# nep-pack/NonlinearEigenproblems.jl

Measured on AMD Instinct MI355X. Metric: eigenpairs/sec (gun SPMF iar m=100) + compute_Mlincomb GB/s, higher is better.
Workload: dtype f64 (complex128)

## Files before the change

include/nepmi355.h:

```cpp
#ifndef NEPMI355_H
#define NEPMI355_H

#include <stddef.h>
#include <stdint.h>

#ifdef __cplusplus
extern "C" {
#endif

typedef struct { double re, im; } nep_cdouble;
typedef struct nep_spmf nep_spmf;
typedef struct nep_lu nep_lu;
typedef struct nep_comm nep_comm;
typedef void* nep_stream;

#define NEP_OK 0
#define NEP_ERR_HIP -1
#define NEP_ERR_ARG -2
#define NEP_ERR_SINGULAR -3
#define NEP_ERR_BREAKDOWN -4
#define NEP_ERR_UNSUPPORTED -5
#define NEP_ERR_RETRY -6
#define NEP_ERR_NOCONV -7

// ... 261 lines not shown
    double tol;
    double neigs;
    nep_cdouble sigma, gamma;
} nep_iar_opts;
typedef struct nep_iar_result {
    int32_t k;
    int32_t nconv;
    int32_t nret;
    int32_t refine_plan;
    int32_t refine_hint_off;
    int32_t retry_reason;
} nep_iar_result;
typedef int32_t (*nep_fv_eval)(void* ctx, int32_t nlam, const nep_cdouble* lam, nep_cdouble* F);
int32_t nep_refine_review(int32_t umfpack_refinements, int32_t plan, int32_t final_recorded, const double* w4, int32_t hint_in,
                          int32_t out[4]);
int32_t nep_iar_run(nep_spmf* spmf, nep_lu* lu, int64_t n, const nep_iar_opts* opts, const nep_cdouble* h_v0,
                    const nep_cdouble* h_Ctab, int32_t mt, const double* h_cabs, const nep_cdouble* h_cf, const double* h_fro,
                    nep_fv_eval fv, void* ctx, nep_cdouble* h_lam, nep_cdouble* dQ, nep_cdouble* h_Q, double* h_err,
                    nep_cdouble* dV_basis, nep_iar_result* res, nep_stream stream);

int32_t nep_comm_unique_id(void* h_out128);
int32_t nep_comm_create(int32_t rank, int32_t world, const void* h_unique_id128, nep_comm** out);
int32_t nep_comm_destroy(nep_comm* c);
int32_t nep_comm_info(const nep_comm* c, int32_t out[2]);
int32_t nep_allgather_sum(nep_comm* c, const nep_cdouble* d_partial, int64_t len, nep_cdouble* d_total, nep_stream stream);
int32_t nep_sum_ranks(const nep_cdouble* d_parts, int64_t len, int32_t world, nep_cdouble* d_total, nep_stream stream);

#ifdef __cplusplus
}
#endif
// ... 2 lines not shown
```

nonlineareigenproblems.jl_amd/_lib.py:

```python
import ctypes as C
import os

import numpy as np
import torch

from ._env import env_flag

_HERE = os.path.dirname(os.path.abspath(__file__))
LIB_PATH = os.path.join(_HERE, "libnepmi355.so")


class NepError(RuntimeError):
    def __init__(self, status, msg):
        super().__init__("libnepmi355 status %d: %s" % (status, msg))
        self.status = status


NEP_OK, NEP_ERR_HIP, NEP_ERR_ARG, NEP_ERR_SINGULAR, NEP_ERR_BREAKDOWN, NEP_ERR_UNSUPPORTED = 0, -1, -2, -3, -4, -5
NEP_ERR_RETRY, NEP_ERR_NOCONV = -6, -7


def _load():
    from . import build
    if build.needs_build():
# ... 124 lines not shown
    "nep_lu_refac_destroy": [c_vp],
    "nep_lu_refac_info": [c_vp, c_vp],
    "nep_lu_refac_wide_info": [c_vp, c_vp],
    "nep_lu_refac_hash": [c_vp, c_vp],
    "nep_lu_factor_dev": [c_vp, c_vp, c_i32, C.c_double, c_vp, c_vp, c_vp, c_vp],
    "nep_lu_refac_analyze": [c_i64, c_vp, c_vp, c_vp, c_vp, c_vp, c_vp, c_vp, c_vp, c_vp],
    "nep_lu_factor_dev_batch": [c_vp, c_i32, c_vp, c_i32, C.c_double, c_vp, c_vp, c_vp, c_vp],
    "nep_lu_factor_dev_batch_terms": [c_vp, c_i32, c_vp, c_i32, c_vp, c_i32, C.c_double, c_vp, c_vp, c_vp],
    "nep_iar_step": [c_vp, c_i32, c_i32, c_vp],
    "nep_iar_steps": [c_vp, c_i32, c_i32, c_i32, c_vp],
    "nep_iar_wait": [c_vp, c_i32],
    "nep_iar_stream_wait": [c_vp, c_i32, c_vp],
    "nep_devprim_exclusive_sum": [c_vp, c_vp, c_i64, c_vp],
    "nep_devprim_sort_pairs": [c_vp, c_vp, c_i64, c_i32, c_vp],
    "nep_refine_review": [c_i32, c_i32, c_i32, c_vp, c_i32, c_vp],
    "nep_iar_run": [c_vp, c_vp, c_i64, c_vp, c_vp, c_vp, c_i32, c_vp, c_vp, c_vp, c_vp, c_vp, c_vp, c_vp, c_vp, c_vp, c_vp, c_vp, c_vp],
    "nep_hess_eig_worksize": [c_i32, P(c_i64)],
    "nep_hess_eigvals_dev": [c_i32, c_vp, c_i64, c_vp, c_vp, c_vp, c_vp],
    "nep_hess_eigvecs_dev": [c_i32, c_vp, c_vp, c_i64, c_vp, c_vp, c_vp],
    "nep_hess_eigvals_batch_dev": [c_i32, c_i32, c_i32, c_vp, c_i64, c_vp, c_i64, c_vp, c_i64, c_vp, c_i64, c_vp],
    "nep_hess_eigvecs_batch_dev": [c_i32, c_i32, c_i32, c_vp, c_i64, c_vp, c_i64, c_i64, c_vp, c_i64, c_vp, c_i64, c_vp],
    "nep_comm_unique_id": [c_vp],
    "nep_comm_create": [c_i32, c_i32, c_vp, P(c_vp)],
    "nep_comm_destroy": [c_vp],
    "nep_comm_info": [c_vp, P(c_i32)],
    "nep_allgather_sum": [c_vp, c_vp, c_i64, c_vp, c_vp],
    "nep_sum_ranks": [c_vp, c_i64, c_i32, c_vp, c_vp],
    "nep_iar_shift_scale": [c_i64, c_i32, c_vp, c_vp, c_vp],
    "nep_rk_bw": [c_i64, c_i32, c_vp, c_vp, c_vp, c_vp],
    "nep_discretize_polygon": [c_i32, c_vp, c_i32, c_vp],
# ... 64 lines not shown
```

nonlineareigenproblems.jl_amd/csrc/driver.hip:

```cpp
#include "common.h"
#include <vector>
#include <stdlib.h>
#include <time.h>

struct nep_iar {
    nep_spmf* spmf; nep_lu* lu;
    int64_t n, ldv; int32_t m, mt;
    cplx* dV; const cplx* dCtab; int64_t ldc; const int64_t* d_active;
    cplx* dz; cplx* dW;
    std::vector<double> cabs; std::vector<nep_cdouble> cf;
    cplx* dH; nep_cdouble* hH;
    double* d_cabs; cplx* d_ccf;
    cplx* hH_dev;
    int32_t method;
    std::vector<hipEvent_t> ev;
    hipEvent_t e_upload = nullptr; bool upload_waited = false;
    hipStream_t last = nullptr;
    bool no_events = false;
    std::vector<hipGraphExec_t> graphs;
    cplx* dWT = nullptr; int32_t wt_for = 0;
};

extern "C" {

int32_t nep_iar_create(nep_spmf* spmf, nep_lu* lu, int64_t n, int32_t m, nep_cdouble* dV, int64_t ldv,
                       const nep_cdouble* dCtab, int64_t ldc, const int64_t* d_active, nep_cdouble* dwork3n,
                       const double* h_cabs, const nep_cdouble* h_cf, int32_t mt, nep_cdouble* dH, nep_cdouble* h_pinnedH,
                       int32_t orth_method, nep_iar** out) {
    ARGCHK(out != nullptr);
    *out = nullptr;
// ... 95 lines not shown
        if (rc) return rc;
    }
    cplx* mirror = s->hH_dev ? s->hH_dev + (int64_t)(k - 1) * (s->m + 4) : nullptr;
    if (s->dWT && k < s->m) {
        rc = nep_orth_dev_iar_next((const nep_cdouble*)s->dV, s->ldv, n, k, s->d_active, (nep_cdouble*)vv, (nep_cdouble*)hrow, s->method,
                                   (nep_cdouble*)mirror, k + 4, (const nep_cdouble*)s->dCtab, s->ldc, s->mt,
                                   (nep_cdouble*)s->dWT, (nep_cdouble*)(vv + s->ldv + n), stream);
        if (!rc) s->wt_for = k + 1;
    } else
        rc = nep_orth_dev_mirror((const nep_cdouble*)s->dV, s->ldv, n * (int64_t)(k + 1), k, s->d_active, (nep_cdouble*)vv,
                                 (nep_cdouble*)hrow, s->method, (nep_cdouble*)mirror, k + 4, stream);
    if (rc) return rc;
    if (!mirror)
        HIPCHK(hipMemcpyAsync(s->hH + (int64_t)(k - 1) * (s->m + 4), hrow, (size_t)(k + 4) * sizeof(cplx), hipMemcpyDeviceToHost, st));
    if (s->no_events) return NEP_OK;
    if (!s->ev[k]) HIPCHK(hipEventCreateWithFlags(&s->ev[k], hipEventDisableTiming | hipEventBlockingSync));
    HIPCHK(hipEventRecord(s->ev[k], st));
    return NEP_OK;
}

int32_t nep_iar_steps(nep_iar* s, int32_t k0, int32_t count, int32_t refine_steps, nep_stream stream) {
    ARGCHK(s && count >= 1);
    for (int32_t k = k0; k < k0 + count; ++k) {
        int rc = nep_iar_step(s, k, refine_steps, stream);
        if (rc) return rc;
    }
    return NEP_OK;
}

int32_t nep_iar_steps_graph(nep_iar* s, int32_t k0, int32_t count, int32_t refine_steps, nep_stream stream, int32_t* captured) {
    ARGCHK(s && count >= 1);
    if (captured) *captured = 0;
// ... 8 lines not shown
        hipGraph_t g = nullptr;
        hipError_t e = hipStreamEndCapture(st, &g);
        hipGraphExec_t ge = nullptr;
        if (!rc && e == hipSuccess && g && hipGraphInstantiate(&ge, g, nullptr, nullptr, 0) == hipSuccess && ge) {
            if (hipGraphLaunch(ge, st) == hipSuccess) { s->graphs.push_back(ge); ok = true; }
            else (void)hipGraphExecDestroy(ge);
        }
        if (g) (void)hipGraphDestroy(g);
        if (!ok) (void)hipGetLastError();
    } else (void)hipGetLastError();
    if (!ok) {
        s->wt_for = wt_for0; s->upload_waited = waited0; s->last = last0;
        return nep_iar_steps(s, k0, count, refine_steps, stream);
    }
    for (int32_t k = k0; k < k0 + count; ++k) {
        if (!s->ev[k]) HIPCHK(hipEventCreateWithFlags(&s->ev[k], hipEventDisableTiming | hipEventBlockingSync));
        HIPCHK(hipEventRecord(s->ev[k], st));
    }
    if (captured) *captured = 1;
    return NEP_OK;
}

int32_t nep_iar_wait(nep_iar* s, int32_t k) {
    ARGCHK(s && k >= 1 && k <= s->m && s->ev[k]);
    for (;;) {
        const hipError_t e = hipEventQuery(s->ev[k]);
        if (e == hipSuccess) return NEP_OK;
        if (e != hipErrorNotReady) HIPCHK(e);
        struct timespec ts = {0, 20000};
        nanosleep(&ts, nullptr);
// ... 11 lines not shown
```

nonlineareigenproblems.jl_amd/csrc/iar_run.hip:

```cpp
#include "common.h"
#include <algorithm>
#include <deque>
#include <map>
#include <mutex>
#include <vector>
#include <math.h>
#include <time.h>

extern "C" {
int32_t nep_iar_create(nep_spmf* spmf, nep_lu* lu, int64_t n, int32_t m, nep_cdouble* dV, int64_t ldv, const nep_cdouble* dCtab,
                       int64_t ldc, const int64_t* d_active, nep_cdouble* dwork3n, const double* h_cabs, const nep_cdouble* h_cf,
                       int32_t mt, nep_cdouble* dH, nep_cdouble* h_pinnedH, int32_t orth_method, nep_iar** out);
int32_t nep_iar_steps_graph(nep_iar* s, int32_t k0, int32_t count, int32_t refine_steps, nep_stream stream, int32_t* captured);
}

namespace {

constexpr double EPS = 2.220446049250313e-16;

__global__ void k_iar_active(int64_t* act, int64_t n, int m1) {
    const int j = blockIdx.x * blockDim.x + threadIdx.x;
    if (j < m1) act[j] = (int64_t)(j + 1) * n;
}
__global__ void k_iar_start(cplx* __restrict__ V, const cplx* __restrict__ v, double inv, int64_t n) {
    const int64_t i = (int64_t)blockIdx.x * blockDim.x + threadIdx.x;
    if (i < n) V[i] = cmake(v[i].x * inv, v[i].y * inv);
}

// ... 40 lines not shown
    RunStreams& r = g_rs[dev];
    if (!r.check || !r.eig || r.probed_for != main || (r.shared && r.retries < 3)) {
        if (r.shared) ++r.retries;
        r.shared = false;
        int rc = pick_stream(r.check, {main}, &r.check, &r.shared); if (rc) return rc;
        rc = pick_stream(r.eig, {main, r.check}, &r.eig, &r.shared); if (rc) return rc;
        r.probed_for = main;
    }
    *out = r;
    return NEP_OK;
}

struct Arena {
    int dev = -1; int64_t n = 0; int32_t m = 0, mt = 0;
    cplx* Hdev = nullptr; cplx* wdev = nullptr; cplx* Ctab = nullptr; cplx* work3n = nullptr; int64_t* active = nullptr;
    cplx* v0 = nullptr; double* d_norms = nullptr; void* eigwork = nullptr; int64_t wsz = 0; int bmax = 0;
    cplx* Hpin = nullptr; cplx* wpin = nullptr; double* npin = nullptr; cplx* stage = nullptr;
    void release() {
        for (void* p : {(void*)Hdev, (void*)wdev, (void*)Ctab, (void*)work3n, (void*)active, (void*)v0, (void*)d_norms, eigwork})
            if (p) nep_pool_free(p);
        for (void* p : {(void*)Hpin, (void*)wpin, (void*)npin, (void*)stage}) if (p) (void)hipHostFree(p);
        *this = Arena();
    }
};
std::mutex g_arena_mu;
std::vector<Arena> g_arenas;

int arena_acquire(int64_t n, int32_t m, int32_t mt, int bmax, Arena* out) {
    int dev = 0; HIPCHK(hipGetDevice(&dev));
    {
        std::lock_guard<std::mutex> lk(g_arena_mu);
        for (size_t i = 0; i < g_arenas.size(); ++i)
            if (g_arenas[i].dev == dev && g_arenas[i].n == n && g_arenas[i].m == m && g_arenas[i].mt == mt && g_arenas[i].bmax == bmax) {
                *out = g_arenas[i]; g_arenas.erase(g_arenas.begin() + i); return NEP_OK;
            }
    }
    Arena a; a.dev = dev; a.n = n; a.m = m; a.mt = mt; a.bmax = bmax;
    int64_t wsz = 0; int rc = nep_hess_eig_worksize(m, &wsz); if (rc) return rc;
    a.wsz = (wsz + 15) / 16 * 16;
    void* p = nullptr;
#define AL(dst, type, bytes) do { rc = nep_pool_alloc(&p, (size_t)(bytes)); if (rc) { a.release(); return rc; } dst = (type)p; } while (0)
    AL(a.Hdev, cplx*, (size_t)m * (m + 4) * 16);
    AL(a.wdev, cplx*, (size_t)m * (m + 2) * 16);
    AL(a.Ctab, cplx*, (size_t)m * mt * 16);
    AL(a.work3n, cplx*, (size_t)3 * n * 16);
    AL(a.active, int64_t*, (size_t)(m + 1) * 8);
    AL(a.v0, cplx*, (size_t)n * 16);
    AL(a.d_norms, double*, (size_t)m * 2 * m * 8);
    AL(a.eigwork, void*, (size_t)bmax * a.wsz);
#undef AL
    const size_t stage_bytes = std::max<size_t>((size_t)n * 16, (size_t)m * mt * 16);
    if (hipHostMalloc((void**)&a.Hpin, (size_t)m * (m + 4) * 16, hipHostMallocMapped) != hipSuccess ||
        hipHostMalloc((void**)&a.wpin, (size_t)m * (m + 2) * 16, hipHostMallocMapped) != hipSuccess ||
        hipHostMalloc((void**)&a.npin, (size_t)m * 2 * m * 8, hipHostMallocDefault) != hipSuccess ||
        hipHostMalloc((void**)&a.stage, stage_bytes, hipHostMallocDefault) != hipSuccess) {
        (void)hipGetLastError(); a.release();
        nep_set_error("nep_iar_run: pinned host allocation failed");
        return NEP_ERR_HIP;
    }
    *out = a;
    return NEP_OK;
}
void arena_return(Arena& a) {
    std::lock_guard<std::mutex> lk(g_arena_mu);
// ... 29 lines not shown
            const double om = w[step];
            if (om <= 2.0 * EPS) { ret = step; break; }
            if (om > 0.5 * w_prev) { ret = om > w_prev ? step - 1 : step; break; }
            if (step == umf) { ret = step; break; }
            w_prev = om;
        }
        if (ret < 0) ret = plan;
        last_omega = w[plan];
        recorded = std::max(ret, 1);
        const bool ok = isfinite(w[plan]) && (ret == plan || w[plan] <= std::max(4.0 * EPS, w[ret]));
        if (ok) { if (!hint_off) hint = recorded; } else { hint = -1; hint_off = true; }
        return ok;
    }
};

struct Batch { std::vector<int> kcs; cplx* Zb = nullptr; int kmax = 0; hipEvent_t evW = nullptr, evZ = nullptr; };
struct Check { int kc = 0; std::vector<double> lam; cplx* QT = nullptr; std::vector<double> F; hipEvent_t ev = nullptr; cplx* Zb_owner = nullptr; };

inline cplx hc(const nep_cdouble& z) { cplx r; r.x = z.re; r.y = z.im; return r; }
inline bool ev_done(hipEvent_t e) {
    if (hipEventQuery(e) == hipSuccess) return true;
    (void)hipGetLastError();
    return false;
}

struct Run {
    nep_spmf* spmf; nep_lu* lu; int64_t n; nep_iar_opts o; nep_fv_eval fv; void* ctx; const double* h_fro;
    hipStream_t st; RunStreams rs; Arena a; bool have_arena = false;
    int32_t m, mt; int64_t ldv;
    cplx* V = nullptr; bool own_V = true; nep_iar* step = nullptr;
    Refine ref;
    std::vector<char> filled; std::vector<int> plans;
    std::vector<hipEvent_t> ev_pool;
    std::vector<double> s_lam; std::vector<int> s_idx; cplx* s_QT = nullptr; int s_kq = 0; int conv = 0; int k_checked = 0;
    std::vector<double> s_err;
    double* h_err = nullptr;
    int retry = 0;

    hipEvent_t event() {
        if (!ev_pool.empty()) { hipEvent_t e = ev_pool.back(); ev_pool.pop_back(); return e; }
        hipEvent_t e = nullptr;
        if (hipEventCreateWithFlags(&e, hipEventDisableTiming) != hipSuccess) { (void)hipGetLastError(); return nullptr; }
        return e;
    }
    void done(hipEvent_t e) { if (e) ev_pool.push_back(e); }

    int fail_kind = 0, fail_at = 0;
    int fill_H(int kk) {
        for (int j = 1; j <= kk; ++j) {
            if (filled[j]) continue;
            if (fail_at == j && (fail_kind == 1 || fail_kind == 2)) {
                retry = fail_kind; nep_set_error("nep_iar_run: injected miss of kind %d at step %d", fail_kind, j); return NEP_ERR_RETRY;
// ... 5 lines not shown
            if (ref.umf > 0) {
                const int plan = plans[j];
                const bool final_rec = !((plan & 0x100) && (j % 8) != 0);
                if (!ref.review((const double*)(row + j + 2), plan & 0xff, final_rec)) {
                    retry = 1; nep_set_error("nep_iar_run: the refinement record of step %d asks for more sweeps than were taken", j);
                    return NEP_ERR_RETRY;
                }
            }
            filled[j] = 1;
        }
        return NEP_OK;
    }
    ~Run() {
        if (step) (void)nep_iar_destroy(step);
        if (V && own_V) nep_pool_free_on(V, st, true);
        if (s_QT) nep_pool_free_on(s_QT, rs.check, true);
        for (hipEvent_t e : ev_pool) (void)hipEventDestroy(e);
        if (have_arena) arena_return(a);
    }
};

}

extern "C" {

int32_t nep_refine_review(int32_t umfpack_refinements, int32_t plan, int32_t final_recorded, const double* w4, int32_t hint_in,
                          int32_t out[4]) {
    ARGCHK(w4 && out && plan >= 0 && plan <= 3 && umfpack_refinements >= 0);
    Refine r; r.umf = umfpack_refinements; r.hint = hint_in;
    const bool ok = r.review(w4, plan, final_recorded != 0);
    out[0] = ok ? 1 : 0; out[1] = r.recorded; out[2] = r.hint; out[3] = r.hint_off ? 1 : 0;
    return NEP_OK;
}

int32_t nep_iar_run(nep_spmf* spmf, nep_lu* lu, int64_t n, const nep_iar_opts* opts, const nep_cdouble* h_v0,
                    const nep_cdouble* h_Ctab, int32_t mt, const double* h_cabs, const nep_cdouble* h_cf, const double* h_fro,
                    nep_fv_eval fv, void* ctx, nep_cdouble* h_lam, nep_cdouble* dQ, nep_cdouble* h_Q, double* h_err,
                    nep_cdouble* dV_basis, nep_iar_result* res, nep_stream stream) {
    ARGCHK(spmf && lu && opts && h_v0 && h_Ctab && fv && h_lam && res);
    ARGCHK(n > 0 && mt >= 1 && opts->maxit >= 1 && opts->check_error_every >= 1);
    ARGCHK(opts->orth_method == 0 || opts->orth_method == 1);
    ARGCHK(opts->errmeasure == 0 || (opts->errmeasure == 1 && h_fro));
    ARGCHK(opts->umfpack_refinements <= 0 || (h_cabs && h_cf));
    memset(res, 0, sizeof(*res));
    res->refine_plan = -1;
    struct timespec t_e_; clock_gettime(CLOCK_MONOTONIC, &t_e_);
    const double t_entry = t_e_.tv_sec * 1e3 + t_e_.tv_nsec * 1e-6;
    const int32_t m = opts->maxit;
    if (m > 128) { nep_set_error("nep_iar_run: maxit = %d exceeds the device eigen-decomposition's limit 128", m); return NEP_ERR_UNSUPPORTED; }
    const int BMAX = std::max(1, nep_env_int("NEP_IAR_EIG_BATCH", 16));
    const int LASTB = std::max(1, nep_env_int("NEP_IAR_EIG_LAST", 8));
    const double T100 = nep_env_double("NEP_IAR_EIG_MS100", 3.3);
    const double TSTEP = 0.35;
    const int cee = opts->check_error_every;
    const double neigs = opts->neigs;
    const bool unthrottled = isinf(neigs) && neigs > 0;

    Run R; R.spmf = spmf; R.lu = lu; R.n = n; R.o = *opts; R.fv = fv; R.ctx = ctx; R.h_fro = h_fro; R.st = as_stream(stream);
    R.m = m; R.mt = mt; R.ldv = n * (int64_t)(m + 1); R.h_err = h_err;
    int rc = run_streams(R.st, &R.rs); if (rc) return rc;
    rc = arena_acquire(n, m, mt, BMAX, &R.a); if (rc) return rc;
    R.have_arena = true;
    Arena& a = R.a;
    hipStream_t st = R.st, cst = R.rs.check, est = R.rs.eig;
    R.ref.umf = opts->umfpack_refinements > 0 ? opts->umfpack_refinements : 0;
    R.ref.hint = (opts->refine_hint >= 0 && nep_env_int("NEP_REFINE_HINT", 1) != 0) ? opts->refine_hint : -1;
    R.filled.assign(m + 1, 0); R.plans.assign(m + 1, 0);
    if (const char* fa = getenv("NEP_IAR_RUN_FAIL_AT")) { if (sscanf(fa, "%d:%d", &R.fail_kind, &R.fail_at) != 2) R.fail_kind = R.fail_at = 0; }
    if (h_err) for (int64_t i = 0; i < (int64_t)m * m; ++i) h_err[i] = NAN;

    if (dV_basis) { R.V = (cplx*)dV_basis; R.own_V = false; }
    else {
        void* p = nullptr;
        rc = nep_pool_alloc(&p, (size_t)(m + 1) * R.ldv * 16); if (rc) return rc;
        R.V = (cplx*)p;
    }
// ... 12 lines not shown
    HIPCHK(hipMemsetAsync(a.Hdev, 0, (size_t)m * (m + 4) * 16, st));
    LAUNCHCHK();
    memset(a.Hpin, 0, (size_t)m * (m + 4) * 16);
    memset(a.wpin, 0, (size_t)m * (m + 2) * 16);
    {
        static thread_local PinnedRing ring;
        rc = ring.upload(a.Ctab, h_Ctab, (size_t)m * mt * 16, st); if (rc) return rc;
    }
    rc = nep_iar_create(spmf, lu, n, m, (nep_cdouble*)R.V, R.ldv, (const nep_cdouble*)a.Ctab, m, a.active, (nep_cdouble*)a.work3n,
                        R.ref.umf > 0 ? h_cabs : nullptr, R.ref.umf > 0 ? h_cf : nullptr, mt, (nep_cdouble*)a.Hdev,
                        (nep_cdouble*)a.Hpin, opts->orth_method, &R.step);
    if (rc) return rc;

    std::vector<char> plan_end(m + 2, 0);
    if (unthrottled) {
        std::vector<int> allk;
        for (int kk = 1; kk <= m; ++kk) if (kk % cee == 0 || kk == m) allk.push_back(kk);
        int e_ = (int)allk.size(); int size = std::min(LASTB, e_);
        while (e_ > 0) {
            plan_end[allk[e_ - 1]] = 1; e_ -= size;
            if (e_ > 0) {
                const double q = allk[e_ - 1] / 100.0;
                size = (int)std::min<double>(std::min(BMAX, e_), std::max(1.0, ceil(2.0 * T100 * q * q / (TSTEP * cee))));
            }
        }
    }
    const bool trace = getenv("NEP_IAR_RUN_TRACE") != nullptr;
    auto now = []() { struct timespec t; clock_gettime(CLOCK_MONOTONIC, &t); return t.tv_sec * 1e3 + t.tv_nsec * 1e-6; };
    double t_fv = 0;
    std::deque<int> pendA; std::deque<Batch> stA; std::deque<Check> stC;
    int slots = unthrottled ? m + 1 : std::max(BMAX, 4);
    const int CHUNK = unthrottled ? 8 : 4;
    const int P = std::min(256, std::max(1, 3072 / mt));
    int k = 1; bool done = false; int status = NEP_OK;
    const bool use_graph = nep_env_flag("NEP_IAR_GRAPH");
    int n_graph = 0;
    auto finished = [&]() { return R.conv >= neigs; };

    auto batch_ready = [&]() -> int {
        if (pendA.empty()) return 0;
        int cnt = 1;
        while (cnt < (int)pendA.size() && cnt < BMAX && pendA[cnt] - pendA[cnt - 1] == pendA[1] - pendA[0] && !(unthrottled && plan_end[pendA[cnt - 1]])) ++cnt;
        if (!unthrottled || plan_end[pendA[cnt - 1]] || cnt >= BMAX || done) return cnt;
        return 0;
    };
    auto launch_batch = [&](int count) -> int {
        Batch b;
        for (int i = 0; i < count; ++i) { b.kcs.push_back(pendA.front()); pendA.pop_front(); }
        const int k0 = b.kcs[0], nb = count; b.kmax = b.kcs.back();
        const int kstep = nb > 1 ? b.kcs[1] - k0 : 0;
        int r = nep_iar_stream_wait(R.step, b.kmax, (nep_stream)est); if (r) return r;
        cplx* wrow = a.wdev + (int64_t)(k0 - 1) * (m + 2);
        cplx* mrow = a.wpin + (int64_t)(k0 - 1) * (m + 2);
        r = nep_hess_eigvals_batch_dev(nb, k0, kstep, (const nep_cdouble*)a.Hdev, m + 4, (nep_cdouble*)wrow, (int64_t)kstep * (m + 2),
                                       a.eigwork, a.wsz, (nep_cdouble*)mrow, (int64_t)kstep * (m + 2), (nep_stream)est);
        if (r) return r;
        b.evW = R.event(); if (!b.evW) return NEP_ERR_HIP;
        HIPCHK(hipEventRecord(b.evW, est));
        void* pz = nullptr;
        r = nep_pool_alloc(&pz, (size_t)nb * b.kmax * b.kmax * 16); if (r) return r;
        b.Zb = (cplx*)pz;
        r = nep_hess_eigvecs_batch_dev(nb, k0, kstep, (nep_cdouble*)wrow, (int64_t)kstep * (m + 2), (nep_cdouble*)b.Zb, b.kmax,
                                       (int64_t)b.kmax * b.kmax, a.eigwork, a.wsz, (nep_cdouble*)mrow, (int64_t)kstep * (m + 2), (nep_stream)est);
        if (r) { nep_pool_free_on(b.Zb, est, true); return r; }
        b.evZ = R.event(); if (!b.evZ) return NEP_ERR_HIP;
        HIPCHK(hipEventRecord(b.evZ, est));
        stA.push_back(b);
        return NEP_OK;
    };
    auto launch_check = [&](const Batch& b, int bi, bool first_of_batch) -> int {
        const int kc = b.kcs[bi];
        int r = R.fill_H(kc); if (r) return r;
        const cplx* w = a.wpin + (int64_t)(kc - 1) * (m + 2);
        if (w[kc].x != 0.0 || (R.fail_kind == 3 && R.fail_at == kc)) { R.retry = 3; nep_set_error("nep_iar_run: the QR iteration of step %d gave up", kc); return NEP_ERR_RETRY; }
        Check c; c.kc = kc; c.lam.resize(2 * (size_t)kc); c.F.resize(2 * (size_t)mt * kc);
        const double sr = R.o.sigma.re, si = R.o.sigma.im, gr = R.o.gamma.re, gi = R.o.gamma.im;
        for (int s = 0; s < kc; ++s) {
            const double dr = w[s].x, di = w[s].y, den = dr * dr + di * di;
            c.lam[2 * s] = sr + (gr * dr + gi * di) / den;
            c.lam[2 * s + 1] = si + (gi * dr - gr * di) / den;
        }
        const double tf0 = trace ? now() : 0.0;
        const int32_t frc = R.fv(R.ctx, kc, (const nep_cdouble*)c.lam.data(), (nep_cdouble*)c.F.data());
        if (trace) t_fv += now() - tf0;
        if (frc != 0) {
            nep_set_error("nep_iar_run: the f_t(lambda) callback failed in step %d", kc); return NEP_ERR_ARG;
        }
        if (first_of_batch) HIPCHK(hipStreamWaitEvent(cst, b.evZ, 0));
        void* pq = nullptr;
        r = nep_pool_alloc(&pq, (size_t)n * kc * 16); if (r) return r;
        c.QT = (cplx*)pq;
        r = nep_gemm_ts_dev((const nep_cdouble*)R.V, R.ldv, n, kc, (const nep_cdouble*)(b.Zb + (int64_t)bi * b.kmax * b.kmax), b.kmax, 0, kc,
                            (nep_cdouble*)c.QT, kc, 1, (nep_stream)cst);
        double* d_out = a.d_norms + (int64_t)(kc - 1) * 2 * m;
        if (!r) r = nep_resid_batch_dev(spmf, kc, (const nep_cdouble*)c.F.data(), (const nep_cdouble*)c.QT, kc, d_out, (nep_stream)cst);
        if (r) { nep_pool_free_on(c.QT, cst, true); return r; }
        HIPCHK(hipMemcpyAsync(a.npin + (int64_t)(kc - 1) * 2 * m, d_out, (size_t)2 * kc * 8, hipMemcpyDeviceToHost, cst));
        c.ev = R.event(); if (!c.ev) return NEP_ERR_HIP;
        HIPCHK(hipEventRecord(c.ev, cst));
        if (bi == (int)b.kcs.size() - 1) c.Zb_owner = b.Zb;
        stC.push_back(std::move(c));
        return NEP_OK;
    };
    auto consume = [&](Check& c) -> int {
        const int kc = c.kc;
        const cplx* w = a.wpin + (int64_t)(kc - 1) * (m + 2);
        if (w[kc + 1].x != 0.0) { R.retry = 3; nep_set_error("nep_iar_run: an inverse iteration of step %d did not grow", kc); return NEP_ERR_RETRY; }
        const double* sq = a.npin + (int64_t)(kc - 1) * 2 * m;
        std::vector<double> e(kc);
        for (int j0 = 0; j0 < kc; j0 += P) {
            const int kk = std::min(P, kc - j0);
            for (int j = 0; j < kk; ++j) {
                const double rn = sqrt(sq[2 * j0 + j]), qn = sqrt(sq[2 * j0 + kk + j]);
                double den = qn;
                if (R.o.errmeasure == 1) {
// ... 11 lines not shown
        std::stable_sort(idx.begin(), idx.end(), [&](int x, int y) {
            const double ex = isnan(e[x]) ? INFINITY : e[x], ey = isnan(e[y]) ? INFINITY : e[y];
            return ex < ey;
        });
        R.s_err.assign(kc, 0.0);
        for (int s = 0; s < kc; ++s) R.s_err[s] = e[idx[s]];
        if (R.h_err) for (int s = 0; s < kc; ++s) R.h_err[(int64_t)s * m + (kc - 1)] = R.s_err[s];
        int nret = kc;
        if (kc == m || conv >= neigs) nret = (int)std::min<double>(kc, neigs);
        R.s_lam.resize(2 * (size_t)nret); R.s_idx.assign(idx.begin(), idx.begin() + nret);
        for (int s = 0; s < nret; ++s) {
            const int src = (kc == m || conv >= neigs) ? idx[s] : s;
            R.s_lam[2 * s] = c.lam[2 * src]; R.s_lam[2 * s + 1] = c.lam[2 * src + 1];
        }
        if (!(kc == m || conv >= neigs)) for (int s = 0; s < nret; ++s) R.s_idx[s] = idx[s];
        if (R.s_QT) nep_pool_free_on(R.s_QT, cst, true);
        R.s_QT = c.QT; c.QT = nullptr; R.s_kq = kc;
        R.conv = conv; R.k_checked = kc;
        R.done(c.ev); c.ev = nullptr;
        return NEP_OK;
    };
    auto drop_check = [&](Check& c) {
        if (c.QT) nep_pool_free_on(c.QT, cst, true);
        if (c.Zb_owner) nep_pool_free_on(c.Zb_owner, cst, true);
        R.done(c.ev);
    };
    auto drop_batch = [&](Batch& b) {
        if (b.Zb) nep_pool_free_on(b.Zb, est, true);
        R.done(b.evW); R.done(b.evZ);
    };

    hipEvent_t te0 = nullptr, te1 = nullptr; bool te1_rec = false;
    if (trace) { (void)hipEventCreate(&te0); (void)hipEventCreate(&te1); (void)hipEventRecord(te0, st); }
    const double t_loop = now();
    double tt_steps = 0, tt_A = 0, tt_B = 0, tt_C = 0, tt_sleep = 0, t_enq_done = 0; double tq = 0;
    while (status == NEP_OK) {
        bool progressed = false;
        tq = now();
        if (!done) {
            if (k <= m && !finished()) {
                int nb = 0;
                while (nb < CHUNK && k + nb <= m) {
                    const bool due = ((k + nb) % cee == 0) || (k + nb == m);
// ... 5 lines not shown
                    if (plan > 0 && R.ref.settled()) plan |= 0x100;
                    if (use_graph && k > 1) { int32_t cap = 0; status = nep_iar_steps_graph(R.step, k, nb, plan, stream, &cap); n_graph += cap; }
                    else status = nep_iar_steps(R.step, k, nb, plan, stream);
                    if (status) break;
                    for (int kk = k; kk < k + nb; ++kk) {
                        R.plans[kk] = plan;
                        if (kk % cee == 0 || kk == m) pendA.push_back(kk);
                    }
                    k += nb; progressed = true;
                }
            } else done = true;
            if (k > m) { if (!done && trace) { t_enq_done = now() - t_loop; if (te1 && !te1_rec) { (void)hipEventRecord(te1, st); te1_rec = true; } } done = true; }
        }
        if (trace) { const double t = now(); tt_steps += t - tq; tq = t; }
        while (!finished()) {
            const int cnt = batch_ready();
            if (!cnt) break;
            status = launch_batch(cnt); progressed = true;
            if (status) break;
        }
        if (status) break;
        if (trace) { const double t = now(); tt_A += t - tq; tq = t; }
        while (!stA.empty() && !finished() && ev_done(stA.front().evW)) {
            progressed = true;
            Batch b = stA.front(); stA.pop_front();
            for (int bi = 0; bi < (int)b.kcs.size() && status == NEP_OK; ++bi) {
                status = launch_check(b, bi, bi == 0);
                if (status == NEP_OK) ++slots;
            }
            if (status) { drop_batch(b); break; }
            R.done(b.evW); R.done(b.evZ);
        }
        if (status) break;
        if (trace) { const double t = now(); tt_B += t - tq; tq = t; }
        while (!stC.empty() && !finished() && ev_done(stC.front().ev)) {
            progressed = true;
            Check c = std::move(stC.front()); stC.pop_front();
            status = consume(c);
            if (c.Zb_owner) nep_pool_free_on(c.Zb_owner, cst, true);
            c.Zb_owner = nullptr;
            if (status) { drop_check(c); break; }
        }
        if (status) break;
        if (finished()) {
            done = true; pendA.clear();
            while (!stA.empty()) { drop_batch(stA.front()); stA.pop_front(); }
            while (!stC.empty()) { drop_check(stC.front()); stC.pop_front(); }
        }
        if (trace) { const double t = now(); tt_C += t - tq; tq = t; }
        if (done && pendA.empty() && stA.empty() && stC.empty()) break;
        if (!progressed) { struct timespec ts = {0, 20000}; nanosleep(&ts, nullptr); if (trace) { const double t = now(); tt_sleep += t - tq; tq = t; } }
    }
    if (trace)
        fprintf(stderr, "nep_iar_run trace (ms): set-up %.2f | loop %.2f: steps %.2f (all enqueued at %.2f) A %.2f B %.2f (callback %.2f) C %.2f sleep %.2f\n",
// ... 15 lines not shown
    res->refine_plan = R.ref.hint_off ? -1 : (R.ref.recorded >= 0 ? R.ref.recorded : R.ref.hint);
    res->refine_hint_off = R.ref.hint_off ? 1 : 0;
    if (status || !unthrottled) (void)hipStreamSynchronize(st);
    if (status) return status;

    int nret = (int)(R.s_lam.size() / 2);
    const bool noconv = (R.conv < neigs) && !unthrottled;
    if (!noconv) nret = std::min(nret, R.conv);
    res->k = R.k_checked > 0 ? R.k_checked : k - 1;
    res->nconv = R.conv; res->nret = nret;
    for (int s = 0; s < nret; ++s) { h_lam[s].re = R.s_lam[2 * s]; h_lam[s].im = R.s_lam[2 * s + 1]; }
    if (nret > 0 && (dQ || h_Q) && R.s_QT) {
        cplx* dst = (cplx*)dQ; void* tmp = nullptr;
        if (!dst) { rc = nep_pool_alloc(&tmp, (size_t)n * nret * 16); if (rc) return rc; dst = (cplx*)tmp; }
        std::vector<int32_t> cols(R.s_idx.begin(), R.s_idx.begin() + nret);
        rc = nep_rowmajor_to_colmajor(n, R.s_kq, (const nep_cdouble*)R.s_QT, R.s_kq, cols.data(), nret, (nep_cdouble*)dst, n, (nep_stream)cst);
        if (!rc && h_Q) {
            if (hipMemcpyAsync(h_Q, dst, (size_t)n * nret * 16, hipMemcpyDeviceToHost, cst) != hipSuccess) rc = NEP_ERR_HIP;
        }
        if (hipStreamSynchronize(cst) != hipSuccess && !rc) rc = NEP_ERR_HIP;
        if (tmp) nep_pool_free(tmp);
        if (rc) { if (rc == NEP_ERR_HIP) nep_set_error("nep_iar_run: returning the eigenvector block failed"); return rc; }
    }
    if (noconv) { nep_set_error("Number of iterations exceeded. maxit=%d.", m); return NEP_ERR_NOCONV; }
    return NEP_OK;
}

}
```

nonlineareigenproblems.jl_amd/csrc/util.hip:

```cpp
#include "common.h"
#include <vector>
#include <algorithm>
#include <math.h>
#include <time.h>

static thread_local char g_err[1024] = "";

void nep_set_error(const char* fmt, ...) {
    va_list ap;
    va_start(ap, fmt);
    vsnprintf(g_err, sizeof(g_err), fmt, ap);
    va_end(ap);
}

int NepScratch::ensure(size_t bytes) {
    if (bytes <= cap) return NEP_OK;
    if (dptr) { (void)hipDeviceSynchronize(); nep_pool_free(dptr); dptr = nullptr; cap = 0; }
    size_t want = std::max<size_t>(2 * bytes, (size_t)4 << 20);
    int rc = nep_pool_alloc(&dptr, want);
    if (rc) return rc;
    cap = want;
    return NEP_OK;
}
void NepScratch::release() {
// ... 97 lines not shown
        *p = busy_p;
        return NEP_OK;
    }
    {
        std::vector<PoolBlock> to_free;
        {
            std::lock_guard<std::mutex> lk(g_pool_mu);
            for (auto& kv : g_pool_free) to_free.push_back(kv.second);
            g_pool_free.clear(); g_pool_cached = 0;
        }
        pool_drop(to_free);
    }
    HIPCHK(hipMalloc(p, want));
    std::lock_guard<std::mutex> lk(g_pool_mu);
    g_pool_live[*p] = want;
    return NEP_OK;
}

void nep_pool_free(void* p) {
    if (!p) return;
    std::vector<PoolBlock> to_free;
    {
        std::lock_guard<std::mutex> lk(g_pool_mu);
        pool_put(p, nullptr, to_free);
    }
    pool_drop(to_free);
}

void nep_pool_free_on(void* p, hipStream_t st, bool in_flight) {
    if (!p) return;
// ... 643 lines not shown
```

Before: 1404.

## Run IAR eigen-check batches on alternating stream lanes with sparse step events

Eigenvalue/eigenvector batches and their residual checks now alternate between two stream lanes (eig and check), with the final step on the main stream. Each lane has its own eigen workspace slot, and event chaining orders the checks. Step events are recorded only at batch-end steps, and the batch plan splits off the last check. The aim is to let consecutive Hessenberg eig batches and residual checks overlap and to cut per-step event overhead. The cost is a larger workspace, more complex stream ordering, and a risk of ordering bugs.

```diff
diff --git a/include/nepmi355.h b/include/nepmi355.h
--- a/include/nepmi355.h
+++ b/include/nepmi355.h
@@ -299,6 +299,7 @@
 typedef int32_t (*nep_fv_eval)(void* ctx, int32_t nlam, const nep_cdouble* lam, nep_cdouble* F);
 int32_t nep_refine_review(int32_t umfpack_refinements, int32_t plan, int32_t final_recorded, const double* w4, int32_t hint_in,
                           int32_t out[4]);
+int32_t nep_iar_batch_plan(int32_t m, int32_t check_error_every, int32_t bmax, int32_t lastb, double ms100, char* out_end_flags);
 int32_t nep_iar_run(nep_spmf* spmf, nep_lu* lu, int64_t n, const nep_iar_opts* opts, const nep_cdouble* h_v0,
                     const nep_cdouble* h_Ctab, int32_t mt, const double* h_cabs, const nep_cdouble* h_cf, const double* h_fro,
                     nep_fv_eval fv, void* ctx, nep_cdouble* h_lam, nep_cdouble* dQ, nep_cdouble* h_Q, double* h_err,
diff --git a/nonlineareigenproblems.jl_amd/_lib.py b/nonlineareigenproblems.jl_amd/_lib.py
--- a/nonlineareigenproblems.jl_amd/_lib.py
+++ b/nonlineareigenproblems.jl_amd/_lib.py
@@ -162,6 +162,7 @@
     "nep_devprim_exclusive_sum": [c_vp, c_vp, c_i64, c_vp],
     "nep_devprim_sort_pairs": [c_vp, c_vp, c_i64, c_i32, c_vp],
     "nep_refine_review": [c_i32, c_i32, c_i32, c_vp, c_i32, c_vp],
+    "nep_iar_batch_plan": [c_i32, c_i32, c_i32, c_i32, C.c_double, c_vp],
     "nep_iar_run": [c_vp, c_vp, c_i64, c_vp, c_vp, c_vp, c_i32, c_vp, c_vp, c_vp, c_vp, c_vp, c_vp, c_vp, c_vp, c_vp, c_vp, c_vp, c_vp],
     "nep_hess_eig_worksize": [c_i32, P(c_i64)],
     "nep_hess_eigvals_dev": [c_i32, c_vp, c_i64, c_vp, c_vp, c_vp, c_vp],
diff --git a/nonlineareigenproblems.jl_amd/csrc/driver.hip b/nonlineareigenproblems.jl_amd/csrc/driver.hip
--- a/nonlineareigenproblems.jl_amd/csrc/driver.hip
+++ b/nonlineareigenproblems.jl_amd/csrc/driver.hip
@@ -14,6 +14,7 @@
     cplx* hH_dev;
     int32_t method;
     std::vector<hipEvent_t> ev;
+    std::vector<char> ev_wanted;
     hipEvent_t e_upload = nullptr; bool upload_waited = false;
     hipStream_t last = nullptr;
     bool no_events = false;
@@ -139,8 +140,15 @@
     if (!mirror)
         HIPCHK(hipMemcpyAsync(s->hH + (int64_t)(k - 1) * (s->m + 4), hrow, (size_t)(k + 4) * sizeof(cplx), hipMemcpyDeviceToHost, st));
     if (s->no_events) return NEP_OK;
+    if (!s->ev_wanted.empty() && !s->ev_wanted[k]) return NEP_OK;
     if (!s->ev[k]) HIPCHK(hipEventCreateWithFlags(&s->ev[k], hipEventDisableTiming | hipEventBlockingSync));
     HIPCHK(hipEventRecord(s->ev[k], st));
+    return NEP_OK;
+}
+
+int32_t nep_iar_event_steps(nep_iar* s, const char* wanted) {
+    ARGCHK(s);
+    if (wanted) s->ev_wanted.assign(wanted, wanted + s->m + 1); else s->ev_wanted.clear();
     return NEP_OK;
 }
 
@@ -179,6 +187,7 @@
         return nep_iar_steps(s, k0, count, refine_steps, stream);
     }
     for (int32_t k = k0; k < k0 + count; ++k) {
+        if (!s->ev_wanted.empty() && !s->ev_wanted[k]) continue;
         if (!s->ev[k]) HIPCHK(hipEventCreateWithFlags(&s->ev[k], hipEventDisableTiming | hipEventBlockingSync));
         HIPCHK(hipEventRecord(s->ev[k], st));
     }
diff --git a/nonlineareigenproblems.jl_amd/csrc/iar_run.hip b/nonlineareigenproblems.jl_amd/csrc/iar_run.hip
--- a/nonlineareigenproblems.jl_amd/csrc/iar_run.hip
+++ b/nonlineareigenproblems.jl_amd/csrc/iar_run.hip
@@ -12,6 +12,7 @@
                        int64_t ldc, const int64_t* d_active, nep_cdouble* dwork3n, const double* h_cabs, const nep_cdouble* h_cf,
                        int32_t mt, nep_cdouble* dH, nep_cdouble* h_pinnedH, int32_t orth_method, nep_iar** out);
 int32_t nep_iar_steps_graph(nep_iar* s, int32_t k0, int32_t count, int32_t refine_steps, nep_stream stream, int32_t* captured);
+int32_t nep_iar_event_steps(nep_iar* s, const char* wanted);
 }
 
 namespace {
@@ -82,7 +83,7 @@
 struct Arena {
     int dev = -1; int64_t n = 0; int32_t m = 0, mt = 0;
     cplx* Hdev = nullptr; cplx* wdev = nullptr; cplx* Ctab = nullptr; cplx* work3n = nullptr; int64_t* active = nullptr;
-    cplx* v0 = nullptr; double* d_norms = nullptr; void* eigwork = nullptr; int64_t wsz = 0; int bmax = 0;
+    cplx* v0 = nullptr; double* d_norms = nullptr; void* eigwork = nullptr; int64_t wsz = 0; int bmax = 0; int nslots = 0;
     cplx* Hpin = nullptr; cplx* wpin = nullptr; double* npin = nullptr; cplx* stage = nullptr;
     void release() {
         for (void* p : {(void*)Hdev, (void*)wdev, (void*)Ctab, (void*)work3n, (void*)active, (void*)v0, (void*)d_norms, eigwork})
@@ -94,16 +95,16 @@
 std::mutex g_arena_mu;
 std::vector<Arena> g_arenas;
 
-int arena_acquire(int64_t n, int32_t m, int32_t mt, int bmax, Arena* out) {
+int arena_acquire(int64_t n, int32_t m, int32_t mt, int bmax, int nslots, Arena* out) {
     int dev = 0; HIPCHK(hipGetDevice(&dev));
     {
         std::lock_guard<std::mutex> lk(g_arena_mu);
         for (size_t i = 0; i < g_arenas.size(); ++i)
-            if (g_arenas[i].dev == dev && g_arenas[i].n == n && g_arenas[i].m == m && g_arenas[i].mt == mt && g_arenas[i].bmax == bmax) {
+            if (g_arenas[i].dev == dev && g_arenas[i].n == n && g_arenas[i].m == m && g_arenas[i].mt == mt && g_arenas[i].bmax == bmax && g_arenas[i].nslots == nslots) {
                 *out = g_arenas[i]; g_arenas.erase(g_arenas.begin() + i); return NEP_OK;
             }
     }
-    Arena a; a.dev = dev; a.n = n; a.m = m; a.mt = mt; a.bmax = bmax;
+    Arena a; a.dev = dev; a.n = n; a.m = m; a.mt = mt; a.bmax = bmax; a.nslots = nslots;
     int64_t wsz = 0; int rc = nep_hess_eig_worksize(m, &wsz); if (rc) return rc;
     a.wsz = (wsz + 15) / 16 * 16;
     void* p = nullptr;
@@ -115,7 +116,7 @@
     AL(a.active, int64_t*, (size_t)(m + 1) * 8);
     AL(a.v0, cplx*, (size_t)n * 16);
     AL(a.d_norms, double*, (size_t)m * 2 * m * 8);
-    AL(a.eigwork, void*, (size_t)bmax * a.wsz);
+    AL(a.eigwork, void*, (size_t)nslots * a.wsz);
 #undef AL
     const size_t stage_bytes = std::max<size_t>((size_t)n * 16, (size_t)m * mt * 16);
     if (hipHostMalloc((void**)&a.Hpin, (size_t)m * (m + 4) * 16, hipHostMallocMapped) != hipSuccess ||
@@ -175,8 +176,28 @@
     }
 };
 
-struct Batch { std::vector<int> kcs; cplx* Zb = nullptr; int kmax = 0; hipEvent_t evW = nullptr, evZ = nullptr; };
-struct Check { int kc = 0; std::vector<double> lam; cplx* QT = nullptr; std::vector<double> F; hipEvent_t ev = nullptr; cplx* Zb_owner = nullptr; };
+struct Batch { std::vector<int> kcs; cplx* Zb = nullptr; int kmax = 0; hipEvent_t evW = nullptr, evZ = nullptr;
+               hipStream_t sd = nullptr, sc = nullptr; int lane = -1; };
+struct Check { int kc = 0; std::vector<double> lam; cplx* QT = nullptr; std::vector<double> F; hipEvent_t ev = nullptr; cplx* Zb_owner = nullptr;
+               hipStream_t st = nullptr; };
+
+void batch_plan(int m, int cee, int bmax, int lastb, double ms100, bool split_last, char* end_flags) {
+    const double TSTEP = 0.35;
+    std::vector<int> allk;
+    for (int kk = 1; kk <= m; ++kk) if (kk % cee == 0 || kk == m) allk.push_back(kk);
+    int e_ = (int)allk.size(); int size = std::min(std::min(lastb, bmax), e_);
+    if (split_last) {
+        end_flags[allk[e_ - 1]] = 1; --e_;
+        size = std::min(std::min(std::max(lastb - 1, 1), bmax), e_);
+    }
+    while (e_ > 0) {
+        end_flags[allk[e_ - 1]] = 1; e_ -= size;
+        if (e_ > 0) {
+            const double q = allk[e_ - 1] / 100.0;
+            size = (int)std::min<double>(std::min(bmax, e_), std::max(1.0, ceil(2.0 * ms100 * q * q / (TSTEP * cee))));
+        }
+    }
+}
 
 inline cplx hc(const nep_cdouble& z) { cplx r; r.x = z.re; r.y = z.im; return r; }
 inline bool ev_done(hipEvent_t e) {
@@ -193,10 +214,11 @@
     Refine ref;
     std::vector<char> filled; std::vector<int> plans;
     std::vector<hipEvent_t> ev_pool;
-    std::vector<double> s_lam; std::vector<int> s_idx; cplx* s_QT = nullptr; int s_kq = 0; int conv = 0; int k_checked = 0;
+    std::vector<double> s_lam; std::vector<int> s_idx; cplx* s_QT = nullptr; hipStream_t s_st = nullptr; int s_kq = 0; int conv = 0; int k_checked = 0;
     std::vector<double> s_err;
     double* h_err = nullptr;
     int retry = 0;
+    hipEvent_t chain[3] = {nullptr, nullptr, nullptr};
 
     hipEvent_t event() {
         if (!ev_pool.empty()) { hipEvent_t e = ev_pool.back(); ev_pool.pop_back(); return e; }
@@ -232,8 +254,9 @@
     ~Run() {
         if (step) (void)nep_iar_destroy(step);
         if (V && own_V) nep_pool_free_on(V, st, true);
-        if (s_QT) nep_pool_free_on(s_QT, rs.check, true);
+        if (s_QT) nep_pool_free_on(s_QT, s_st, true);
         for (hipEvent_t e : ev_pool) (void)hipEventDestroy(e);
+        for (hipEvent_t e : chain) if (e) (void)hipEventDestroy(e);
         if (have_arena) arena_return(a);
     }
 };
@@ -248,6 +271,13 @@
     Refine r; r.umf = umfpack_refinements; r.hint = hint_in;
     const bool ok = r.review(w4, plan, final_recorded != 0);
     out[0] = ok ? 1 : 0; out[1] = r.recorded; out[2] = r.hint; out[3] = r.hint_off ? 1 : 0;
+    return NEP_OK;
+}
+
+int32_t nep_iar_batch_plan(int32_t m, int32_t check_error_every, int32_t bmax, int32_t lastb, double ms100, char* out_end_flags) {
+    ARGCHK(out_end_flags && m >= 1 && check_error_every >= 1 && bmax >= 1 && lastb >= 1 && ms100 > 0.0);
+    memset(out_end_flags, 0, (size_t)m + 2);
+    batch_plan(m, check_error_every, bmax, lastb, ms100, true, out_end_flags);
     return NEP_OK;
 }
 
@@ -269,7 +299,8 @@
     const int BMAX = std::max(1, nep_env_int("NEP_IAR_EIG_BATCH", 16));
     const int LASTB = std::max(1, nep_env_int("NEP_IAR_EIG_LAST", 8));
     const double T100 = nep_env_double("NEP_IAR_EIG_MS100", 3.3);
-    const double TSTEP = 0.35;
+    const bool lanes = nep_env_int("NEP_IAR_LANES", 1) != 0;
+    const bool all_events = nep_env_int("NEP_IAR_STEP_EVENTS", 0) != 0;
     const int cee = opts->check_error_every;
     const double neigs = opts->neigs;
     const bool unthrottled = isinf(neigs) && neigs > 0;
@@ -277,7 +308,7 @@
     Run R; R.spmf = spmf; R.lu = lu; R.n = n; R.o = *opts; R.fv = fv; R.ctx = ctx; R.h_fro = h_fro; R.st = as_stream(stream);
     R.m = m; R.mt = mt; R.ldv = n * (int64_t)(m + 1); R.h_err = h_err;
     int rc = run_streams(R.st, &R.rs); if (rc) return rc;
-    rc = arena_acquire(n, m, mt, BMAX, &R.a); if (rc) return rc;
+    rc = arena_acquire(n, m, mt, BMAX, lanes ? 2 * BMAX + 1 : BMAX, &R.a); if (rc) return rc;
     R.have_arena = true;
     Arena& a = R.a;
     hipStream_t st = R.st, cst = R.rs.check, est = R.rs.eig;
@@ -320,17 +351,17 @@
 
     std::vector<char> plan_end(m + 2, 0);
     if (unthrottled) {
-        std::vector<int> allk;
-        for (int kk = 1; kk <= m; ++kk) if (kk % cee == 0 || kk == m) allk.push_back(kk);
-        int e_ = (int)allk.size(); int size = std::min(LASTB, e_);
-        while (e_ > 0) {
-            plan_end[allk[e_ - 1]] = 1; e_ -= size;
-            if (e_ > 0) {
-                const double q = allk[e_ - 1] / 100.0;
-                size = (int)std::min<double>(std::min(BMAX, e_), std::max(1.0, ceil(2.0 * T100 * q * q / (TSTEP * cee))));
-            }
-        }
-    }
+        batch_plan(m, cee, BMAX, LASTB, T100, lanes, plan_end.data());
+        if (!all_events) {
+            std::vector<char> wanted(plan_end.begin(), plan_end.begin() + m + 1);
+            if (lanes) wanted[m] = 0;
+            else if (m % cee != 0 && m > cee) wanted[m / cee * cee] = 1;
+            rc = nep_iar_event_steps(R.step, wanted.data()); if (rc) return rc;
+        }
+    }
+    if (lanes) for (hipEvent_t& e : R.chain) HIPCHK(hipEventCreateWithFlags(&e, hipEventDisableTiming));
+    hipStream_t lane_st[3] = {est, cst, st};
+    bool lane_busy[2] = {false, false}; int last_lane = 1; int chk_lane = -1;
     const bool trace = getenv("NEP_IAR_RUN_TRACE") != nullptr;
     auto now = []() { struct timespec t; clock_gettime(CLOCK_MONOTONIC, &t); return t.tv_sec * 1e3 + t.tv_nsec * 1e-6; };
     double t_fv = 0;
@@ -343,34 +374,49 @@
     int n_graph = 0;
     auto finished = [&]() { return R.conv >= neigs; };
 
-    auto batch_ready = [&]() -> int {
+    auto batch_ready = [&](int* lane) -> int {
+        *lane = -1;
         if (pendA.empty()) return 0;
         int cnt = 1;
-        while (cnt < (int)pendA.size() && cnt < BMAX && pendA[cnt] - pendA[cnt - 1] == pendA[1] - pendA[0] && !(unthrottled && plan_end[pendA[cnt - 1]])) ++cnt;
-        if (!unthrottled || plan_end[pendA[cnt - 1]] || cnt >= BMAX || done) return cnt;
-        return 0;
+        while (cnt < (int)pendA.size() && cnt < BMAX && pendA[cnt] - pendA[cnt - 1] == pendA[1] - pendA[0] && !(unthrottled && plan_end[pendA[cnt - 1]]) &&
+               !(lanes && pendA[cnt] == m)) ++cnt;
+        if (!(!unthrottled || plan_end[pendA[cnt - 1]] || cnt >= BMAX || done)) return 0;
+        if (!lanes) return cnt;
+        if (pendA[0] == m) { *lane = 2; return 1; }
+        const int other = 1 - last_lane;
+        if (!lane_busy[other]) *lane = other; else if (!lane_busy[last_lane]) *lane = last_lane; else return 0;
+        return cnt;
     };
-    auto launch_batch = [&](int count) -> int {
+    auto launch_batch = [&](int count, int lane) -> int {
         Batch b;
         for (int i = 0; i < count; ++i) { b.kcs.push_back(pendA.front()); pendA.pop_front(); }
         const int k0 = b.kcs[0], nb = count; b.kmax = b.kcs.back();
         const int kstep = nb > 1 ? b.kcs[1] - k0 : 0;
-        int r = nep_iar_stream_wait(R.step, b.kmax, (nep_stream)est); if (r) return r;
+        b.lane = lane; b.sd = lane < 0 ? est : lane_st[lane]; b.sc = lane < 0 ? cst : lane_st[lane];
+        void* work = lane <= 0 ? a.eigwork : (void*)((char*)a.eigwork + (size_t)(lane == 1 ? BMAX : 2 * BMAX) * a.wsz);
+        if (lane >= 0 && lane < 2) { lane_busy[lane] = true; last_lane = lane; }
+        int r = NEP_OK;
+        if (lane != 2) { r = nep_iar_stream_wait(R.step, b.kmax, (nep_stream)b.sd); if (r) return r; }
         cplx* wrow = a.wdev + (int64_t)(k0 - 1) * (m + 2);
         cplx* mrow = a.wpin + (int64_t)(k0 - 1) * (m + 2);
         r = nep_hess_eigvals_batch_dev(nb, k0, kstep, (const nep_cdouble*)a.Hdev, m + 4, (nep_cdouble*)wrow, (int64_t)kstep * (m + 2),
-                                       a.eigwork, a.wsz, (nep_cdouble*)mrow, (int64_t)kstep * (m + 2), (nep_stream)est);
+                                       work, a.wsz, (nep_cdouble*)mrow, (int64_t)kstep * (m + 2), (nep_stream)b.sd);
         if (r) return r;
         b.evW = R.event(); if (!b.evW) return NEP_ERR_HIP;
-        HIPCHK(hipEventRecord(b.evW, est));
+        if (hipEventRecord(b.evW, b.sd) != hipSuccess) { (void)hipGetLastError(); R.done(b.evW); nep_set_error("nep_iar_run: hipEventRecord failed"); return NEP_ERR_HIP; }
         void* pz = nullptr;
-        r = nep_pool_alloc(&pz, (size_t)nb * b.kmax * b.kmax * 16); if (r) return r;
+        r = nep_pool_alloc(&pz, (size_t)nb * b.kmax * b.kmax * 16); if (r) { R.done(b.evW); return r; }
         b.Zb = (cplx*)pz;
         r = nep_hess_eigvecs_batch_dev(nb, k0, kstep, (nep_cdouble*)wrow, (int64_t)kstep * (m + 2), (nep_cdouble*)b.Zb, b.kmax,
-                                       (int64_t)b.kmax * b.kmax, a.eigwork, a.wsz, (nep_cdouble*)mrow, (int64_t)kstep * (m + 2), (nep_stream)est);
-        if (r) { nep_pool_free_on(b.Zb, est, true); return r; }
-        b.evZ = R.event(); if (!b.evZ) return NEP_ERR_HIP;
-        HIPCHK(hipEventRecord(b.evZ, est));
+                                       (int64_t)b.kmax * b.kmax, work, a.wsz, (nep_cdouble*)mrow, (int64_t)kstep * (m + 2), (nep_stream)b.sd);
+        if (r) { nep_pool_free_on(b.Zb, b.sd, true); R.done(b.evW); return r; }
+        if (!lanes) {
+            b.evZ = R.event(); if (!b.evZ) { nep_pool_free_on(b.Zb, b.sd, true); R.done(b.evW); return NEP_ERR_HIP; }
+            if (hipEventRecord(b.evZ, b.sd) != hipSuccess) {
+                (void)hipGetLastError(); nep_pool_free_on(b.Zb, b.sd, true); R.done(b.evW); R.done(b.evZ);
+                nep_set_error("nep_iar_run: hipEventRecord failed"); return NEP_ERR_HIP;
+            }
+        }
         stA.push_back(b);
         return NEP_OK;
     };
@@ -392,19 +438,27 @@
         if (frc != 0) {
             nep_set_error("nep_iar_run: the f_t(lambda) callback failed in step %d", kc); return NEP_ERR_ARG;
         }
-        if (first_of_batch) HIPCHK(hipStreamWaitEvent(cst, b.evZ, 0));
+        const hipStream_t cs = b.sc;
+        if (first_of_batch && !lanes) HIPCHK(hipStreamWaitEvent(cs, b.evZ, 0));
+        if (first_of_batch && lanes && chk_lane >= 0 && chk_lane != b.lane) HIPCHK(hipStreamWaitEvent(cs, R.chain[chk_lane], 0));
         void* pq = nullptr;
         r = nep_pool_alloc(&pq, (size_t)n * kc * 16); if (r) return r;
         c.QT = (cplx*)pq;
         r = nep_gemm_ts_dev((const nep_cdouble*)R.V, R.ldv, n, kc, (const nep_cdouble*)(b.Zb + (int64_t)bi * b.kmax * b.kmax), b.kmax, 0, kc,
-                            (nep_cdouble*)c.QT, kc, 1, (nep_stream)cst);
+                            (nep_cdouble*)c.QT, kc, 1, (nep_stream)cs);
         double* d_out = a.d_norms + (int64_t)(kc - 1) * 2 * m;
-        if (!r) r = nep_resid_batch_dev(spmf, kc, (const nep_cdouble*)c.F.data(), (const nep_cdouble*)c.QT, kc, d_out, (nep_stream)cst);
-        if (r) { nep_pool_free_on(c.QT, cst, true); return r; }
-        HIPCHK(hipMemcpyAsync(a.npin + (int64_t)(kc - 1) * 2 * m, d_out, (size_t)2 * kc * 8, hipMemcpyDeviceToHost, cst));
-        c.ev = R.event(); if (!c.ev) return NEP_ERR_HIP;
-        HIPCHK(hipEventRecord(c.ev, cst));
-        if (bi == (int)b.kcs.size() - 1) c.Zb_owner = b.Zb;
+        if (!r) r = nep_resid_batch_dev(spmf, kc, (const nep_cdouble*)c.F.data(), (const nep_cdouble*)c.QT, kc, d_out, (nep_stream)cs);
+        if (r) { nep_pool_free_on(c.QT, cs, true); return r; }
+        c.st = cs;
+        if (hipMemcpyAsync(a.npin + (int64_t)(kc - 1) * 2 * m, d_out, (size_t)2 * kc * 8, hipMemcpyDeviceToHost, cs) != hipSuccess ||
+            !(c.ev = R.event()) || hipEventRecord(c.ev, cs) != hipSuccess) {
+            (void)hipGetLastError(); nep_pool_free_on(c.QT, cs, true); R.done(c.ev);
+            nep_set_error("nep_iar_run: enqueueing the check of step %d failed", kc); return NEP_ERR_HIP;
+        }
+        if (bi == (int)b.kcs.size() - 1) {
+            c.Zb_owner = b.Zb;
+            if (lanes) { HIPCHK(hipEventRecord(R.chain[b.lane], cs)); chk_lane = b.lane; if (b.lane < 2) lane_busy[b.lane] = false; }
+        }
         stC.push_back(std::move(c));
         return NEP_OK;
     };
@@ -446,19 +500,19 @@
             R.s_lam[2 * s] = c.lam[2 * src]; R.s_lam[2 * s + 1] = c.lam[2 * src + 1];
         }
         if (!(kc == m || conv >= neigs)) for (int s = 0; s < nret; ++s) R.s_idx[s] = idx[s];
-        if (R.s_QT) nep_pool_free_on(R.s_QT, cst, true);
-        R.s_QT = c.QT; c.QT = nullptr; R.s_kq = kc;
+        if (R.s_QT) nep_pool_free_on(R.s_QT, R.s_st, true);
+        R.s_QT = c.QT; c.QT = nullptr; R.s_st = c.st; R.s_kq = kc;
         R.conv = conv; R.k_checked = kc;
         R.done(c.ev); c.ev = nullptr;
         return NEP_OK;
     };
     auto drop_check = [&](Check& c) {
-        if (c.QT) nep_pool_free_on(c.QT, cst, true);
-        if (c.Zb_owner) nep_pool_free_on(c.Zb_owner, cst, true);
+        if (c.QT) nep_pool_free_on(c.QT, c.st, true);
+        if (c.Zb_owner) nep_pool_free_on(c.Zb_owner, c.st, true);
         R.done(c.ev);
     };
     auto drop_batch = [&](Batch& b) {
-        if (b.Zb) nep_pool_free_on(b.Zb, est, true);
+        if (b.Zb) nep_pool_free_on(b.Zb, b.sd, true);
         R.done(b.evW); R.done(b.evZ);
     };
 
@@ -494,9 +548,10 @@
         }
         if (trace) { const double t = now(); tt_steps += t - tq; tq = t; }
         while (!finished()) {
-            const int cnt = batch_ready();
+            int lane = -1;
+            const int cnt = batch_ready(&lane);
             if (!cnt) break;
-            status = launch_batch(cnt); progressed = true;
+            status = launch_batch(cnt, lane); progressed = true;
             if (status) break;
         }
         if (status) break;
@@ -517,7 +572,7 @@
             progressed = true;
             Check c = std::move(stC.front()); stC.pop_front();
             status = consume(c);
-            if (c.Zb_owner) nep_pool_free_on(c.Zb_owner, cst, true);
+            if (c.Zb_owner) nep_pool_free_on(c.Zb_owner, c.st, true);
             c.Zb_owner = nullptr;
             if (status) { drop_check(c); break; }
         }
@@ -563,11 +618,12 @@
         cplx* dst = (cplx*)dQ; void* tmp = nullptr;
         if (!dst) { rc = nep_pool_alloc(&tmp, (size_t)n * nret * 16); if (rc) return rc; dst = (cplx*)tmp; }
         std::vector<int32_t> cols(R.s_idx.begin(), R.s_idx.begin() + nret);
-        rc = nep_rowmajor_to_colmajor(n, R.s_kq, (const nep_cdouble*)R.s_QT, R.s_kq, cols.data(), nret, (nep_cdouble*)dst, n, (nep_stream)cst);
+        const hipStream_t xs = R.s_st;
+        rc = nep_rowmajor_to_colmajor(n, R.s_kq, (const nep_cdouble*)R.s_QT, R.s_kq, cols.data(), nret, (nep_cdouble*)dst, n, (nep_stream)xs);
         if (!rc && h_Q) {
-            if (hipMemcpyAsync(h_Q, dst, (size_t)n * nret * 16, hipMemcpyDeviceToHost, cst) != hipSuccess) rc = NEP_ERR_HIP;
-        }
-        if (hipStreamSynchronize(cst) != hipSuccess && !rc) rc = NEP_ERR_HIP;
+            if (hipMemcpyAsync(h_Q, dst, (size_t)n * nret * 16, hipMemcpyDeviceToHost, xs) != hipSuccess) rc = NEP_ERR_HIP;
+        }
+        if (hipStreamSynchronize(xs) != hipSuccess && !rc) rc = NEP_ERR_HIP;
         if (tmp) nep_pool_free(tmp);
         if (rc) { if (rc == NEP_ERR_HIP) nep_set_error("nep_iar_run: returning the eigenvector block failed"); return rc; }
     }
diff --git a/nonlineareigenproblems.jl_amd/csrc/util.hip b/nonlineareigenproblems.jl_amd/csrc/util.hip
--- a/nonlineareigenproblems.jl_amd/csrc/util.hip
+++ b/nonlineareigenproblems.jl_amd/csrc/util.hip
@@ -135,6 +135,15 @@
     HIPCHK(hipMalloc(p, want));
     std::lock_guard<std::mutex> lk(g_pool_mu);
     g_pool_live[*p] = want;
+    return NEP_OK;
+}
+
+extern "C" int32_t nep_pool_stats(int64_t out[2]) {
+    ARGCHK(out);
+    std::lock_guard<std::mutex> lk(g_pool_mu);
+    int64_t live = 0;
+    for (auto& kv : g_pool_live) live += (int64_t)kv.second;
+    out[0] = live; out[1] = (int64_t)g_pool_cached;
     return NEP_OK;
 }
 
```

After: 1447 (median of 4 runs). 1.03x the previous value.
